# placeforyiming/DistanceTransform-DepthCompletion

Hardware: AMD Instinct MI355X
Metric: DT+NN-fill frames/sec at 352x1216; achieved HBM GB/s vs peak (higher is better)
Workload: dtype u32

## Files before the change

distancetransform-depthcompletion_amd/csrc/dtfill_fused.hpp:

```cpp
#pragma once

constexpr int F_NT = 256;
constexpr int F_P = 196;
constexpr int F_NWD = 6;
constexpr int F_HW = 3;
constexpr int F_RS = 7;
constexpr int F_RROWS = F_WHM + 4;
constexpr int F_RPLANE = F_RROWS * F_RS;
constexpr int F_RING = 1 + 4 * 2 * F_RPLANE;
constexpr int F_EB = 8;
constexpr int F_NONE = 2 * 63;
static_assert(F_WWM == 32 * F_NWD, "window width must be six words");
static_assert(F_RING * 4 >= F_WHM * F_P + 256 * 8, "s_par and the un-slicing table must fit in the ring's memory");
static_assert((F_WHM * F_P) % 8 == 0 && F_WHM * F_P >= 4 * (1 + 4 * F_RPLANE), "the table is 8-byte aligned and lies behind the planes of P1b");

template <int T, int ROW, int BACK>
__device__ __forceinline__ void tap_step(const u32 (&src)[5], u32 (&taken)[F_HW], u32 (&C)[6][F_HW]) {
    static_assert(T >= 0 && T < 8 && ROW == code_di(T) && BACK == code_weight(T), "tap T reads row r + di of level t - weight");
#pragma unroll
    for (int i = 0; i < F_HW; ++i) {
        const u32 cand = row_shift<code_dj(T)>(src + i);
        const u32 sel = cand & ~taken[i];
        taken[i] |= cand;
#pragma unroll
        for (int j = 0; j < 6; ++j)
            if (code_enc(T) & (1 << j)) C[j][i] |= sel;
    }
}

template <int T, int ROW>
__device__ __forceinline__ void bwd_tap(const u32 (&a0)[5], const u32 (&a1)[5], const u32 (&a2)[5], const u32 (&dv)[5],
                                        const u32 (&b0)[F_HW], const u32 (&b1)[F_HW], const u32 (&b2)[F_HW],
                                        u32 (&taken)[F_HW], u32 (&C)[6][F_HW]) {
    constexpr int CODE = T | 8, DJ = code_dj(CODE);
    static_assert(T >= 0 && T < 8 && ROW == code_di(CODE), "backward tap T reads row r - di");
#pragma unroll
    for (int i = 0; i < F_HW; ++i) {
        const u32 m = dist_match<code_weight(CODE)>(row_shift<DJ>(a0 + i), row_shift<DJ>(a1 + i), row_shift<DJ>(a2 + i), b0[i], b1[i], b2[i]) &
                      row_shift<DJ>(dv + i);
        const u32 sel = m & ~taken[i];
        taken[i] |= m;
#pragma unroll
        for (int j = 0; j < 6; ++j)
            if (code_enc(CODE) & (1 << j)) C[j][i] |= sel;
    }
}

__device__ __forceinline__ u32 mul_u24_opaque(u32 a, u32 b) {
    u32 r;
    asm("v_mul_u32_u24 %0, %1, %2" : "=v"(r) : "v"(a), "v"(b));
    return r;
}

#ifdef FUSED_PROF
constexpr int F_PROF_SLOTS = 8192;
__device__ unsigned long long g_fused_prof[F_PROF_SLOTS][16];
constexpr int F_TL_WAVES = 1 << 16, F_TL_EV = 32;
__device__ unsigned long long g_fused_tl[F_TL_WAVES][F_TL_EV];
__device__ __forceinline__ unsigned long long fprof_realtime() {
    unsigned long long t;
    __builtin_amdgcn_sched_barrier(0);
    asm volatile("s_memrealtime %0\n\ts_waitcnt lgkmcnt(0)" : "=s"(t) :: "memory");
    __builtin_amdgcn_sched_barrier(0);
    return t;
}
struct FusedProf {
    unsigned long long t[8] = {}, n[8] = {}, tprev = __builtin_readcyclecounter();
    int nev = 0;
    __device__ int wave() const { return (blockIdx.y * gridDim.x + blockIdx.x) * (blockDim.x >> 6) + (threadIdx.x >> 6); }
    __device__ void event(int k) {
        const unsigned long long rt = fprof_realtime();
        if ((threadIdx.x & 63) == 0 && wave() < F_TL_WAVES && nev < F_TL_EV) g_fused_tl[wave()][nev] = rt << 4 | (unsigned)k;
        ++nev;
    }
    __device__ FusedProf() { event(15); }
    __device__ void mark(int k) {
        const unsigned long long t_ = __builtin_readcyclecounter();
        t[k] += t_ - tprev;
        tprev = t_;
        event(k);
    }
    __device__ void flush() {
        const int slot = wave() % F_PROF_SLOTS;
        if ((threadIdx.x & 63) == 0)
            for (int k = 0; k < 8; ++k) {
                atomicAdd(&g_fused_prof[slot][k], t[k]);
                atomicAdd(&g_fused_prof[slot][8 + k], n[k]);
            }
    }
};
#define FPROF(...) __VA_ARGS__
#else
#define FPROF(...)
#endif

__device__ __forceinline__ void ring_load5(const u32 *__restrict__ ring, int slot, int plane, int row, int wb,
                                           u32 (&a)[5]) {
    const u32 *p = ring + 1 + (slot * 2 + plane) * F_RPLANE + row * F_RS + wb - 1;
#pragma unroll
    for (int i = 0; i < 5; ++i) a[i] = p[i];
}
__device__ __forceinline__ void ring_store3(u32 *__restrict__ ring, int slot, int plane, int row, int wb,
                                            const u32 (&w)[F_HW]) {
    u32 *p = ring + 1 + (slot * 2 + plane) * F_RPLANE + row * F_RS + wb;
#pragma unroll
    for (int i = 0; i < F_HW; ++i) p[i] = w[i];
}

template <int FR, int NT, bool EPI, bool STREAM>
__device__ __forceinline__ bool fused_walk_epilogue(
    const u8 *__restrict__ s_par, const short *__restrict__ s_tab, const uint2 *__restrict__ s_rw, int b, int H,
    int W, int th, int tw, int r0, int c0, int wr0, int wc0, int sh, const float *__restrict__ x,
    const float *__restrict__ vlist,
    int *__restrict__ finfo, int nval, int misaligned, int sky0, float *__restrict__ out_depth, float *__restrict__ out_dt,
    int32_t *__restrict__ out_index, int *__restrict__ frame_status, const DepthEpilogue ep, u32 *__restrict__ rowflag
    FPROF(, FusedProf &prof)) {
    const size_t fo = (size_t)b * H * W;
    const float *gbase = misaligned ? vlist + fo : x + fo;
    const u32 dcrop = EPI ? (u32)(ep.row0 * W) << 2 : 0u;
    const u32 tbytes = (u32)((r0 + th) * W) << 2;
    auto uni = [](int v) { return __builtin_amdgcn_readfirstlane(v); };
    const auto rs_d = __builtin_amdgcn_make_buffer_rsrc(out_depth ? out_depth + (size_t)b * (H - ep.row0) * W : nullptr, 0,
                                                        uni(out_depth && tbytes > dcrop ? (int)(tbytes - dcrop) : 0), 0x00020000);
    const auto rs_t = __builtin_amdgcn_make_buffer_rsrc(out_dt ? out_dt + fo : nullptr, 0, uni(out_dt ? (int)tbytes : 0), 0x00020000);
    const auto rs_i = __builtin_amdgcn_make_buffer_rsrc(out_index ? out_index + fo : nullptr, 0, uni(out_index ? (int)tbytes : 0), 0x00020000);
    constexpr u32 OFF_NONE = 0x80000000u;
    const char *tab = reinterpret_cast<const char *>(s_tab);
    auto step_of = [&](int c) { return (int)*reinterpret_cast<const short *>(tab + c); };
    const int src_base = wr0 * W + wc0;
    const int wrest = W - F_P;
    const u32 last_px = (u32)(H * W - 1);
    bool overflow = false;
    auto put = [](__amdgpu_buffer_rsrc_t rs, u32 off, u32 v) { __builtin_amdgcn_raw_buffer_store_b32(v, rs, (int)off, 0, STREAM ? 2 : 0); };
    const int nslots = ((th + F_EB - 1) / F_EB) * tw;
    const float inv_tw = 1.0f / (float)tw;
    const u32 w4 = (u32)W << 2;
    float p_val[F_EB];
#pragma unroll
    for (int e = 0; e < F_EB; ++e) p_val[e] = 0.0f;
    u32 p_o[F_EB];
#pragma unroll
    for (int e = 0; e < F_EB; ++e) p_o[e] = OFF_NONE;
    auto retire = [&]() {
#pragma unroll
        for (int e = 0; e < F_EB; ++e) put(rs_d, p_o[e] - dcrop, __float_as_uint(EPI ? depth_epilogue(p_val[e], ep) : p_val[e]));
    };
    for (int sb = 0; sb < nslots; sb += NT) {
        int pos[F_EB], step[F_EB], code[F_EB];
        u32 o[F_EB], home0;
        FPROF(prof.mark(5); ++prof.n[2]);
        {
            const int L = sb + (int)threadIdx.x, Lc = min(L, nslots - 1);
            const int g = (int)(((float)Lc + 0.5f) * inv_tw);
            const int tc = Lc - __mul24(g, tw), trb = g * F_EB;
            home0 = (u32)(FR + trb) << 16 | (u32)(FR + tc);
            u32 op = L < nslots ? (u32)(__mul24(r0 + trb, W) + c0 + tc) << 2 : OFF_NONE;
            const int pos0 = __mul24(FR + trb, F_P) + FR + tc;
            unsigned long long und = 0;
#pragma unroll
            for (int e = 0; e < F_EB; ++e) {
                pos[e] = pos0 + e * F_P;
                code[e] = s_par[pos[e]];
                und |= __ballot(code[e] == F_NONE);
                o[e] = code[e] != F_NONE ? op : OFF_NONE;
                asm volatile("" : "+v"(o[e]), "+v"(op));
                op += w4;
            }
            if (und) {
                const int nv = L < nslots ? th - trb : 0;
#pragma unroll
                for (int e = 0; e < F_EB; ++e) overflow |= e < nv && code[e] == F_NONE;
            }
        }
        for (int hop = 0; hop < FR + 2; hop += 2) {
#pragma unroll
            for (int e = 0; e < F_EB; ++e) step[e] = step_of(code[e]);
            int moving = 0;
#pragma unroll
            for (int e = 0; e < F_EB; ++e) moving |= step[e];
            if (!__any(moving != 0)) break;
            FPROF(++prof.n[5]);
#pragma unroll
            for (int e = 0; e < F_EB; ++e) pos[e] += step[e];
#pragma unroll
            for (int e = 0; e < F_EB; ++e) code[e] = s_par[pos[e]];
#pragma unroll
            for (int e = 0; e < F_EB; ++e) step[e] = step_of(code[e]);
#pragma unroll
            for (int e = 0; e < F_EB; ++e) pos[e] += step[e];
#pragma unroll
            for (int e = 0; e < F_EB; ++e) code[e] = s_par[pos[e]];
        }
        FPROF(prof.mark(4); for (int e = 0; e < F_EB; ++e) prof.n[3] += __popcll(__ballot(o[e] != OFF_NONE)));
        int pr[F_EB];
        u32 rc[F_EB], goff[F_EB];
        int lab[F_EB];
        constexpr int F_RG = 4;
#pragma unroll
        for (int h = 0; h < F_EB; h += F_RG) {
            int bp[F_RG], ri[F_RG];
            uint2 rw[F_RG];
            static_assert(F_P == 196 && F_WHM * F_P < (1 << 15), "the reciprocal below is F_P's");
#pragma unroll
            for (int k = 0; k < F_RG; ++k) {
                const int e = h + k;
                pr[e] = (int)(__umul24((u32)pos[e], 5350u) >> 20);
                rc[e] = __umul24((u32)pr[e], 65536u - F_P) + (u32)pos[e];
                bp[k] = (int)(rc[e] + (u32)sh);
                ri[k] = pr[e] * 8 + (int)__builtin_amdgcn_ubfe((u32)bp[k], 5u, 3u);
            }
#pragma unroll
            for (int k = 0; k < F_RG; ++k) rw[k] = s_rw[ri[k]];
#pragma unroll
            for (int k = 0; k < F_RG; ++k) lab[h + k] = (int)rw[k].y + __popc(__builtin_amdgcn_ubfe(rw[k].x, 0u, (u32)bp[k]));
        }
        if (!misaligned) {
#pragma unroll
            for (int e = 0; e < F_EB; ++e) {
                u32 t = (u32)(__mul24(pr[e], wrest) + pos[e]);
                asm("" : "+v"(t));
                goff[e] = min((t + (u32)src_base) << 2, last_px << 2);
            }
        } else {
            bool bad = false;
            const int nv = th + FR - (int)(home0 >> 16);
#pragma unroll
            for (int e = 0; e < F_EB; ++e) {
                const DepthIndex di = depth_index_pos(lab[e], nval);
                bad |= o[e] != OFF_NONE && e < nv && !di.ok;
                goff[e] = (di.ok ? min((u32)di.idx, last_px) : 0u) << 2;
            }
            if (bad && out_depth) atomicOr(frame_status + b, DTFILL_FRAME_INDEX_ERROR);
        }
        retire();
#pragma unroll
        for (int e = 0; e < F_EB; ++e) p_val[e] = *reinterpret_cast<const float *>(reinterpret_cast<const char *>(gbase) + goff[e]);
#pragma unroll
        for (int e = 0; e < F_EB; ++e) {
            p_o[e] = o[e];
            put(rs_i, o[e], (u32)lab[e]);
            put(rs_t, o[e], __float_as_uint((float)__builtin_amdgcn_sad_u16(rc[e], home0 + ((u32)e << 16), 0u)));
        }
    }
    FPROF(prof.mark(5));
    retire();
    const bool any = __any(overflow);
    if (any && !EPI) {
        for (int L = threadIdx.x; L < nslots; L += NT) {
            const int g = L / tw, tc = L - g * tw;
            for (int tr = g * F_EB; tr < min(g * F_EB + F_EB, th); ++tr)
                if (s_par[__mul24(FR + tr, F_P) + FR + tc] == F_NONE) {
                    rowflag[(size_t)b * H + r0 + tr] = 1u;
                    if (sky0 > 0 && (r0 + tr == sky0 || r0 + tr == sky0 + 1)) atomicOr(&finfo[b * FI_STRIDE + FI_SKY], SKY_OFF);
                }
        }
    }
    return any;
}

template <int FR, bool EPI, bool STREAM>
__device__ __forceinline__ void fused_body(int tile, bool premarked, int tbase, int nval, int misaligned, int sky0, const u32 *__restrict__ s_bs,
    const u32 *__restrict__ s_far,
    const float *__restrict__ x, const u64 *__restrict__ srcbits, const u16 *__restrict__ wpre_s,
    const u32 *__restrict__ rowbase_s, int *__restrict__ finfo, const float *__restrict__ vlist,
    int H, int W, int Wd, int nty, int TW, int tiles_x, float *__restrict__ out_depth,
    float *__restrict__ out_dt, int32_t *__restrict__ out_index,
    int *__restrict__ fflag, u32 *__restrict__ rowfar, int *__restrict__ frame_status, const DepthEpilogue ep, u32 *__restrict__ s_ring, uint2 *__restrict__ s_rw,
    short *__restrict__ s_tab, u32 (*__restrict__ s_any)[F_NT / 64]) {
    const int tid = threadIdx.x;
    const int b = blockIdx.x;
    const int ty = tile / tiles_x, tx = tile - ty * tiles_x;
    const int TH = tile_row_height(H, tbase, nty);
    int r0 = tbase + ty * TH;
    const int c0 = tx * TW;
    int th = min(TH, H - r0);
    const int tw = min(TW, W - c0);
    if (th <= 0) return;
    if (premarked) {
        const u32 *rowflag = rowfar + (size_t)b * H;
        auto mine = [&](int i) { return s_far ? ((s_far[i >> 5] >> (i & 31)) & 1u) == 0u : rowflag[i] == 0u; };
        if (tid == 0) {
            s_any[0][0] = 0xFFFFFFFFu;
            s_any[0][1] = 0u;
        }
        __syncthreads();
        if (tid < th && mine(r0 + tid)) {
            atomicMin(&s_any[0][0], (u32)tid);
            atomicMax(&s_any[0][1], (u32)tid + 1u);
        }
        __syncthreads();
        const u32 lo = s_any[0][0], hi = s_any[0][1];
        if (hi == 0u) return;
        r0 += (int)lo;
        th = (int)(hi - lo);
    }
    FPROF(FusedProf prof; prof.n[0] = 1);
    const int wr0 = r0 - FR, wc0 = c0 - FR;
    const int WH = th + 2 * FR, WW = tw + 2 * FR;
    const int ca = max(0, -wc0), cb = min(WW, W - wc0);
    const int w0 = wc0 >> 6;
    const int sh = wc0 - 64 * w0;

    const int r = tid & (F_WHM - 1);
    const int hf = tid >> 7;
    const int wb = F_HW * hf;
    u32 M[F_HW], D[F_HW], TM[F_HW];
    {
        const int gi = wr0 + r;
        const bool rowin = r < WH && gi >= 0 && gi < H;
        const int bit0 = sh + 96 * hf;
        const int kw = bit0 >> 6;
        u32 g[7];
#pragma unroll
        for (int k = 0; k < 3; ++k) {
            const int kk = kw + k;
            const int w = w0 + kk;
            u64 sb = 0;
            u32 rk = 0;
            if (rowin && kk < 4 && w >= 0 && w < Wd) {
                const size_t wi = ((size_t)b * H + gi) * Wd + w;
                sb = srcbits[wi];
                rk = (s_bs ? s_bs[gi] : rowbase_s[(size_t)b * H + gi]) + wpre_s[wi];
            }
            g[2 * k] = (u32)sb;
            g[2 * k + 1] = (u32)(sb >> 32);
            const bool mine = hf == 0 ? kk < 2 : (kk >= 2 && kk < 4);
            if (mine) {
                s_rw[r * 8 + 2 * kk] = make_uint2((u32)sb, rk + 1u);
                s_rw[r * 8 + 2 * kk + 1] = make_uint2((u32)(sb >> 32), rk + 1u + (u32)__popc((u32)sb));
            }
        }
        g[6] = 0;
        const int s6 = bit0 & 63;
        const bool hi = s6 & 32;
        const int s5 = s6 & 31;
#pragma unroll
        for (int i = 0; i < F_HW; ++i) {
            const u32 lo_w = hi ? g[i + 1] : g[i], hi_w = hi ? g[i + 2] : g[i + 1];
            const u32 word = s5 ? __builtin_amdgcn_alignbit(hi_w, lo_w, s5) : lo_w;
            const int lo = max(ca - 32 * (wb + i), 0), up = min(cb - 32 * (wb + i), 32);
            u32 m = 0;
            if (rowin && up > lo) m = (up >= 32 ? 0xFFFFFFFFu : ((1u << up) - 1u)) & ~((1u << lo) - 1u);
            M[i] = m;
            D[i] = word & m;
            const int tlo = max(FR - 32 * (wb + i), 0), tup = min(FR + tw - 32 * (wb + i), 32);
            u32 tm = 0;
            if (r >= FR && r < FR + th && tup > tlo) tm = (tup >= 32 ? 0xFFFFFFFFu : ((1u << tup) - 1u)) & ~((1u << tlo) - 1u);
            TM[i] = tm;
        }
    }
    if (s_bs) __syncthreads();
    for (int k = tid; k < F_RING; k += F_NT) s_ring[k] = 0;
    if (tid < 64) {
        const int hi = tid >> 3, lo = tid & 7;
        s_tab[tid] = (hi <= 4 && lo <= 4) ? (short)((hi - 2) * F_P + (lo - 2)) : (short)0;
    }
    __syncthreads();
    ring_store3(s_ring, 0, 0, r + 2, wb, D);
    ring_store3(s_ring, 0, 1, r + 2, wb, D);
    u32 C[6][F_HW];
#pragma unroll
    for (int j = 0; j < 6; ++j)
#pragma unroll
        for (int i = 0; i < F_HW; ++i) C[j][i] = ((18 >> j) & 1) ? D[i] : 0u;
    u32 Dup[F_HW], Ddn[F_HW];
    u32 Dl = 0, Dr = 0;
#pragma unroll
    for (int i = 0; i < F_HW; ++i) Dup[i] = Ddn[i] = 0;
    __syncthreads();
    FPROF(prof.mark(0));

    u32 P0[F_HW], P1[F_HW], P2[F_HW];
#pragma unroll
    for (int i = 0; i < F_HW; ++i) P0[i] = P1[i] = P2[i] = 0;
    for (int t = 1; t <= FR; ++t) {
        FPROF(++prof.n[1]);
        const int s1 = (t - 1) & 3, s2 = (t - 2) & 3, s3 = (t - 3) & 3, sw = t & 3;
        u32 nb[5], e1[5], l1[5], taken[F_HW], Et[F_HW], Lt[F_HW];
        ring_load5(s_ring, s1, 0, r + 2, wb, e1);
        Dl |= e1[0];
        Dr |= e1[4];
        ring_load5(s_ring, s1, 0, r + 1, wb, nb);
#pragma unroll
        for (int i = 0; i < F_HW; ++i) Dup[i] |= nb[i + 1];
        u32 e1d[5];
        ring_load5(s_ring, s1, 0, r + 3, wb, e1d);
        bool nonempty = false;
        {
            const u32 dd[5] = {Dl, D[0], D[1], D[2], Dr};
#pragma unroll
            for (int i = 0; i < F_HW; ++i) {
                Ddn[i] |= e1d[i + 1];
                const u32 dil = row_shift<1>(dd + i) | row_shift<-1>(dd + i) | Dup[i] | Ddn[i];
                Et[i] = dil & ~D[i] & M[i];
                taken[i] = ~Et[i];
                nonempty |= Et[i] != 0;
            }
        }
        ring_load5(s_ring, s3, 1, r + 0, wb, nb);
        tap_step<0, -2, 3>(nb, taken, C);
        tap_step<1, -2, 3>(nb, taken, C);
        {
            u32 l3[5], l2[5];
            ring_load5(s_ring, s3, 1, r + 1, wb, l3);
            ring_load5(s_ring, s2, 1, r + 1, wb, l2);
            ring_load5(s_ring, s1, 1, r + 1, wb, nb);
            tap_step<2, -1, 3>(l3, taken, C);
            tap_step<3, -1, 2>(l2, taken, C);
            tap_step<4, -1, 1>(nb, taken, C);
            tap_step<5, -1, 2>(l2, taken, C);
            tap_step<6, -1, 3>(l3, taken, C);
        }
        ring_load5(s_ring, s1, 1, r + 2, wb, l1);
        tap_step<7, 0, 1>(l1, taken, C);
        {
            const u32 m0 = (t & 1) ? 0xFFFFFFFFu : 0u, m1 = (t & 2) ? 0xFFFFFFFFu : 0u, m2 = (t & 4) ? 0xFFFFFFFFu : 0u;
#pragma unroll
            for (int i = 0; i < F_HW; ++i) {
                Lt[i] = taken[i] & Et[i];
                P0[i] |= Et[i] & m0;
                P1[i] |= Et[i] & m1;
                P2[i] |= Et[i] & m2;
            }
        }
#pragma unroll
        for (int i = 0; i < F_HW; ++i) D[i] |= Et[i];
        ring_store3(s_ring, sw, 0, r + 2, wb, Et);
        ring_store3(s_ring, sw, 1, r + 2, wb, Lt);
        {
            bool open = false;
#pragma unroll
            for (int i = 0; i < F_HW; ++i) open |= (TM[i] & ~D[i]) != 0;
            const u32 flags = (__any(nonempty) ? 1u : 0u) | (__any(open) ? 2u : 0u);
            if ((tid & 63) == 0) s_any[t & 1][tid >> 6] = flags;
            __syncthreads();
            u32 any = 0;
#pragma unroll
            for (int w = 0; w < F_NT / 64; ++w) any |= s_any[t & 1][w];
            if (any != 3u) break;
        }
    }
    FPROF(prof.mark(1));
    __syncthreads();
    uint2 *s_lut = reinterpret_cast<uint2 *>(reinterpret_cast<u8 *>(s_ring) + F_WHM * F_P);
    s_lut[tid] = make_uint2((((u32)tid & 15u) * 0x00204081u) & 0x01010101u, (((u32)tid >> 4) * 0x00204081u) & 0x01010101u);
    ring_store3(s_ring, 0, 0, r + 2, wb, P0);
    ring_store3(s_ring, 0, 1, r + 2, wb, P1);
    ring_store3(s_ring, 1, 0, r + 2, wb, P2);
    ring_store3(s_ring, 1, 1, r + 2, wb, D);
    __syncthreads();
    {
        u32 taken[F_HW], a0[5], a1[5], a2[5], dv[5];
#pragma unroll
        for (int i = 0; i < F_HW; ++i) {
            const u32 live = C[0][i] | C[1][i] | C[2][i] | C[3][i] | C[4][i] | C[5][i];
            taken[i] = ~(D[i] & ~live);
        }
        auto row4 = [&](int row) {
            ring_load5(s_ring, 0, 0, row, wb, a0);
            ring_load5(s_ring, 0, 1, row, wb, a1);
            ring_load5(s_ring, 1, 0, row, wb, a2);
            ring_load5(s_ring, 1, 1, row, wb, dv);
        };
        row4(r + 4);
        bwd_tap<0, 2>(a0, a1, a2, dv, P0, P1, P2, taken, C);
        bwd_tap<1, 2>(a0, a1, a2, dv, P0, P1, P2, taken, C);
        row4(r + 3);
        bwd_tap<2, 1>(a0, a1, a2, dv, P0, P1, P2, taken, C);
        bwd_tap<3, 1>(a0, a1, a2, dv, P0, P1, P2, taken, C);
        bwd_tap<4, 1>(a0, a1, a2, dv, P0, P1, P2, taken, C);
        bwd_tap<5, 1>(a0, a1, a2, dv, P0, P1, P2, taken, C);
        bwd_tap<6, 1>(a0, a1, a2, dv, P0, P1, P2, taken, C);
        row4(r + 2);
        bwd_tap<7, 0>(a0, a1, a2, dv, P0, P1, P2, taken, C);
    }

    FPROF(prof.mark(2));
    u8 *s_par = reinterpret_cast<u8 *>(s_ring);
    __syncthreads();
    {
        u32 *prow = reinterpret_cast<u32 *>(s_par + r * F_P) + wb * 8;
#pragma unroll
        for (int i = 0; i < F_HW; ++i) {
            u32 cj[6];
#pragma unroll
            for (int j = 0; j < 6; ++j) cj[j] = C[j][i] | ~D[i];
#pragma unroll
            for (int q = 0; q < 4; ++q) {
                u32 lo = 0, hi = 0;
#pragma unroll
                for (int j = 0; j < 6; ++j) {
                    const uint2 sp = s_lut[(cj[j] >> (8 * q)) & 0xFFu];
                    lo |= sp.x << (j + 1);
                    hi |= sp.y << (j + 1);
                }
                prow[i * 8 + 2 * q] = lo;
                prow[i * 8 + 2 * q + 1] = hi;
            }
        }
    }
    __syncthreads();
    FPROF(prof.mark(3));

    const bool overflow = fused_walk_epilogue<FR, F_NT, EPI, STREAM>(s_par, s_tab, s_rw, b, H, W, th, tw, r0, c0, wr0, wc0, sh, x, vlist,
                                                        finfo, nval, misaligned, sky0, out_depth, out_dt, out_index, frame_status, ep, rowfar FPROF(, prof));
    if (overflow && (threadIdx.x & 63) == 0) {
        fflag[b] = EPI ? 2 : 1;
        atomicOr(frame_status + b, DTFILL_FRAME_GENERAL_PATH);
    }
    FPROF(prof.mark(6); prof.flush());
}

constexpr size_t F_OFF_RW = (sizeof(u32) * F_RING + 15) & ~(size_t)15, F_OFF_TAB = F_OFF_RW + sizeof(uint2) * F_WHM * 8, F_OFF_ANY = F_OFF_TAB + sizeof(short) * 64,
                 F_LDS_OWN = F_OFF_ANY + sizeof(u32) * 2 * (F_NT / 64);
constexpr size_t F_LDS = F_LDS_OWN;
constexpr int F_RIDE_HMAX = (int)((sizeof(u32) * F_RING - sizeof(FrameScratch)) / (2 * sizeof(u32)));
static_assert(sizeof(FrameScratch) % 4 == 0 && F_NT == 256, "frame_facts runs on the window kernel's 256 threads");

template <bool STREAM, bool EPI>
__global__ __launch_bounds__(F_NT, 4) void k_fused(
    const float *__restrict__ x, const u64 *__restrict__ srcbits, const u16 *__restrict__ wpre_s,
    const u32 *__restrict__ rowbase_s, int *__restrict__ finfo, float *vlist ,
    int H, int W, int Wd, FusedTiles t16, FusedTiles t32, float *__restrict__ out_depth,
    float *__restrict__ out_dt, int32_t *__restrict__ out_index,
    int *__restrict__ route, int *__restrict__ fflag, u32 *__restrict__ rowfar, int *__restrict__ frame_status, const DepthEpilogue ep,
    const FrameArgs fa) {
    __shared__ __attribute__((aligned(16))) unsigned char s_raw[F_LDS];
    u32 *s_ring = reinterpret_cast<u32 *>(s_raw);
    uint2 *s_rw = reinterpret_cast<uint2 *>(s_raw + F_OFF_RW);
    short *s_tab = reinterpret_cast<short *>(s_raw + F_OFF_TAB);
    u32(*s_any)[F_NT / 64] = reinterpret_cast<u32(*)[F_NT / 64]>(s_raw + F_OFF_ANY);
    const int b = blockIdx.x, tile = blockIdx.y;
    int rt, tbase, nval, misaligned, sky0;
    const u32 *s_bs = nullptr, *s_far = nullptr;
    if (fa.ride) {
        if (tile >= fa.ntmin) {
            if (threadIdx.x == 0) s_any[0][0] = (u32)__hip_atomic_load(&route[b], __ATOMIC_RELAXED, __HIP_MEMORY_SCOPE_AGENT);
            __syncthreads();
            const int seen = (int)s_any[0][0];
            const int rs = seen > 0 ? (seen & 0xFF) : 0;
            if (seen != ROUTE_UNKNOWN && !((rs == 16 && tile < t16.ntiles) || (rs == 32 && tile < t32.ntiles))) return;
        }
        FrameScratch &sc = *reinterpret_cast<FrameScratch *>(s_raw);
        u32 *bs = reinterpret_cast<u32 *>(s_raw + sizeof(FrameScratch)), *bv = bs + H;
        u32 *gs = fa.rowbase_s + (size_t)b * H, *gv = fa.rowbase_v + (size_t)b * H;
        const bool pub = tile == 0;
        const FrameFacts ff = frame_facts(fa.rowcnt_s + (size_t)b * H, fa.rowcnt_v + (size_t)b * H, H, W, fa.mode, fa.nty16, fa.nty32, sc, pub,
                                          [&](int i, u32 base_s, u32 base_v) {
                                              bs[i] = base_s;
                                              bv[i] = base_v;
                                              if (pub) {
                                                  gs[i] = base_s;
                                                  gv[i] = base_v;
                                              }
                                          });
        if (pub)
            frame_publish(ff, sc, b, fa.x, fa.valbits, fa.wpre_v, fa.srcbits, fa.wpre_s, fa.ptslist, H, W, Wd, gs, gv, finfo, vlist,
                          fflag, route, frame_status, fa.mode, fa.negflag, rowfar, true);
        else if (ff.misaligned && out_depth && ((ff.r == 16 && tile < t16.ntiles) || (ff.r == 32 && tile < t32.ntiles)))
            value_list(b, fa.x, fa.valbits, fa.wpre_v, H, W, Wd, vlist, [&](int i) { return bv[i]; });
        auto uni = [](int v) { return __builtin_amdgcn_readfirstlane(v); };
        rt = uni(ff.route);
        tbase = uni(ff.tr0);
        nval = uni(ff.nval);
        misaligned = uni(ff.misaligned);
        sky0 = uni(ff.sky);
        s_bs = bs;
        s_far = sc.far[ff.plane];
    } else {
        rt = route[b];
        tbase = finfo[b * FI_STRIDE + FI_TR0];
        nval = finfo[b * FI_STRIDE + FI_NVAL];
        misaligned = finfo[b * FI_STRIDE + FI_MISALIGNED];
        sky0 = finfo[b * FI_STRIDE + FI_SKY] & ~SKY_OFF;
    }
    if (rt == ROUTE_POINTS) return;
    const int r = rt > 0 ? (rt & 0xFF) : 0;
    const bool pre = rt > 0 && (rt & ROUTE_PREMARK);
#define FUSED_CALL(FR_, T_)                                                                                        \
    fused_body<FR_, EPI, STREAM>(tile, pre, tbase, nval, misaligned, sky0, s_bs, s_far, x, srcbits, wpre_s, rowbase_s, finfo, vlist, H, W, Wd, T_.nty, T_.TW, T_.tiles_x, out_depth, out_dt, \
                          out_index, fflag, rowfar, frame_status, ep, s_ring, s_rw, s_tab, s_any)
    if (r == 16 && tile < t16.ntiles)
        FUSED_CALL(16, t16);
    else if (r == 32 && tile < t32.ntiles)
        FUSED_CALL(32, t32);
#undef FUSED_CALL
}
```

distancetransform-depthcompletion_amd/csrc/dtfill_taps.hpp:

```cpp
#pragma once

constexpr int TAP_OFFSET[8][2] = {{-2, -1}, {-2, 1}, {-1, -2}, {-1, -1}, {-1, 0}, {-1, 1}, {-1, 2}, {0, -1}};
constexpr int tap_di(int t) { return TAP_OFFSET[t][0]; }
constexpr int tap_dj(int t) { return TAP_OFFSET[t][1]; }

constexpr bool code_fwd(int code) { return !(code & 8); }
constexpr int code_di(int code) { return code_fwd(code) ? tap_di(code & 7) : -tap_di(code & 7); }
constexpr int code_dj(int code) { return code_fwd(code) ? tap_dj(code & 7) : -tap_dj(code & 7); }
constexpr int code_weight(int code) { return (code_di(code) < 0 ? -code_di(code) : code_di(code)) + (code_dj(code) < 0 ? -code_dj(code) : code_dj(code)); }
constexpr int code_enc(int code) { return (code_di(code) + 2) << 3 | (code_dj(code) + 2); }

constexpr unsigned tap_nibbles(int axis, int t = 0) { return t == 8 ? 0u : (unsigned)(TAP_OFFSET[t][axis] + 2) << (4 * t) | tap_nibbles(axis, t + 1); }
constexpr unsigned TAP_DI_NIB = tap_nibbles(0), TAP_DJ_NIB = tap_nibbles(1);

constexpr void tap_decode(int code, int &di, int &dj) {
    const int sh = (code & 7) * 4;
    di = (int)((TAP_DI_NIB >> sh) & 15u) - 2;
    dj = (int)((TAP_DJ_NIB >> sh) & 15u) - 2;
    if (code & 8) {
        di = -di;
        dj = -dj;
    }
}
```

Before: 419,800.

## Shrink parent-code planes from six bits to four and drop redundant backward taps

Parent pointers are now stored as 4-bit tap codes (16 values) instead of 6-bit (di,dj) encodings. Codes 13 and 14 are reserved for source and undecided, which frees two bit-planes per word in registers and in the un-slicing epilogue. A separate live mask replaces the OR over all planes. Backward taps 5 and 6 are removed because their candidates are shown to be dominated by code 12. The goal is lower register pressure and fewer ALU and LDS lookups, at the cost of a decode table for codes and a correctness argument that rests on the static asserts.

```diff
diff --git a/distancetransform-depthcompletion_amd/csrc/dtfill_fused.hpp b/distancetransform-depthcompletion_amd/csrc/dtfill_fused.hpp
--- a/distancetransform-depthcompletion_amd/csrc/dtfill_fused.hpp
+++ b/distancetransform-depthcompletion_amd/csrc/dtfill_fused.hpp
@@ -8,32 +8,36 @@
 constexpr int F_RROWS = F_WHM + 4;
 constexpr int F_RPLANE = F_RROWS * F_RS;
 constexpr int F_RING = 1 + 4 * 2 * F_RPLANE;
+constexpr int F_NPLANES = 4;
 constexpr int F_EB = 8;
-constexpr int F_NONE = 2 * 63;
+constexpr int F_NONE = 2 * CODE_NONE;
+static_assert(CODE_SOURCE < (1 << F_NPLANES) && CODE_NONE < (1 << F_NPLANES) && !code_wins(CODE_SOURCE) && !code_wins(CODE_NONE), "the reserved codes fit the planes and never win");
 static_assert(F_WWM == 32 * F_NWD, "window width must be six words");
 static_assert(F_RING * 4 >= F_WHM * F_P + 256 * 8, "s_par and the un-slicing table must fit in the ring's memory");
 static_assert((F_WHM * F_P) % 8 == 0 && F_WHM * F_P >= 4 * (1 + 4 * F_RPLANE), "the table is 8-byte aligned and lies behind the planes of P1b");
 
 template <int T, int ROW, int BACK>
-__device__ __forceinline__ void tap_step(const u32 (&src)[5], u32 (&taken)[F_HW], u32 (&C)[6][F_HW]) {
+__device__ __forceinline__ void tap_step(const u32 (&src)[5], u32 (&taken)[F_HW], u32 (&C)[F_NPLANES][F_HW]) {
     static_assert(T >= 0 && T < 8 && ROW == code_di(T) && BACK == code_weight(T), "tap T reads row r + di of level t - weight");
+    static_assert(code_wins(T), "a reserved code is no tap");
 #pragma unroll
     for (int i = 0; i < F_HW; ++i) {
         const u32 cand = row_shift<code_dj(T)>(src + i);
         const u32 sel = cand & ~taken[i];
         taken[i] |= cand;
 #pragma unroll
-        for (int j = 0; j < 6; ++j)
-            if (code_enc(T) & (1 << j)) C[j][i] |= sel;
+        for (int j = 0; j < F_NPLANES; ++j)
+            if (plane_code(T) & (1 << j)) C[j][i] |= sel;
     }
 }
 
 template <int T, int ROW>
 __device__ __forceinline__ void bwd_tap(const u32 (&a0)[5], const u32 (&a1)[5], const u32 (&a2)[5], const u32 (&dv)[5],
                                         const u32 (&b0)[F_HW], const u32 (&b1)[F_HW], const u32 (&b2)[F_HW],
-                                        u32 (&taken)[F_HW], u32 (&C)[6][F_HW]) {
+                                        u32 (&taken)[F_HW], u32 (&C)[F_NPLANES][F_HW]) {
     constexpr int CODE = T | 8, DJ = code_dj(CODE);
     static_assert(T >= 0 && T < 8 && ROW == code_di(CODE), "backward tap T reads row r - di");
+    static_assert(code_wins(CODE), "codes 13 and 14 never select (dtfill_taps.hpp): they mean source and undecided here");
 #pragma unroll
     for (int i = 0; i < F_HW; ++i) {
         const u32 m = dist_match<code_weight(CODE)>(row_shift<DJ>(a0 + i), row_shift<DJ>(a1 + i), row_shift<DJ>(a2 + i), b0[i], b1[i], b2[i]) &
@@ -41,8 +45,8 @@
         const u32 sel = m & ~taken[i];
         taken[i] |= m;
 #pragma unroll
-        for (int j = 0; j < 6; ++j)
-            if (code_enc(CODE) & (1 << j)) C[j][i] |= sel;
+        for (int j = 0; j < F_NPLANES; ++j)
+            if (plane_code(CODE) & (1 << j)) C[j][i] |= sel;
     }
 }
 
@@ -351,18 +355,22 @@
     }
     if (s_bs) __syncthreads();
     for (int k = tid; k < F_RING; k += F_NT) s_ring[k] = 0;
-    if (tid < 64) {
-        const int hi = tid >> 3, lo = tid & 7;
-        s_tab[tid] = (hi <= 4 && lo <= 4) ? (short)((hi - 2) * F_P + (lo - 2)) : (short)0;
+    if (tid < (1 << F_NPLANES)) {
+        int di, dj;
+        code_step(tid, di, dj);
+        s_tab[tid] = (short)(di * F_P + dj);
     }
     __syncthreads();
     ring_store3(s_ring, 0, 0, r + 2, wb, D);
     ring_store3(s_ring, 0, 1, r + 2, wb, D);
-    u32 C[6][F_HW];
-#pragma unroll
-    for (int j = 0; j < 6; ++j)
-#pragma unroll
-        for (int i = 0; i < F_HW; ++i) C[j][i] = ((18 >> j) & 1) ? D[i] : 0u;
+    u32 C[F_NPLANES][F_HW];
+    u32 Lv[F_HW];
+#pragma unroll
+    for (int i = 0; i < F_HW; ++i) {
+        Lv[i] = D[i];
+#pragma unroll
+        for (int j = 0; j < F_NPLANES; ++j) C[j][i] = ((CODE_SOURCE >> j) & 1) ? D[i] : 0u;
+    }
     u32 Dup[F_HW], Ddn[F_HW];
     u32 Dl = 0, Dr = 0;
 #pragma unroll
@@ -373,7 +381,7 @@
     u32 P0[F_HW], P1[F_HW], P2[F_HW];
 #pragma unroll
     for (int i = 0; i < F_HW; ++i) P0[i] = P1[i] = P2[i] = 0;
-    for (int t = 1; t <= FR; ++t) {
+    auto level = [&](const int t) __attribute__((always_inline)) -> bool {
         FPROF(++prof.n[1]);
         const int s1 = (t - 1) & 3, s2 = (t - 2) & 3, s3 = (t - 3) & 3, sw = t & 3;
         u32 nb[5], e1[5], l1[5], taken[F_HW], Et[F_HW], Lt[F_HW];
@@ -418,6 +426,7 @@
 #pragma unroll
             for (int i = 0; i < F_HW; ++i) {
                 Lt[i] = taken[i] & Et[i];
+                Lv[i] |= Lt[i];
                 P0[i] |= Et[i] & m0;
                 P1[i] |= Et[i] & m1;
                 P2[i] |= Et[i] & m2;
@@ -437,9 +446,10 @@
             u32 any = 0;
 #pragma unroll
             for (int w = 0; w < F_NT / 64; ++w) any |= s_any[t & 1][w];
-            if (any != 3u) break;
-        }
-    }
+            return any == 3u;
+        }
+    };
+    for (int t = 1; t <= FR && level(t); ++t) {}
     FPROF(prof.mark(1));
     __syncthreads();
     uint2 *s_lut = reinterpret_cast<uint2 *>(reinterpret_cast<u8 *>(s_ring) + F_WHM * F_P);
@@ -452,10 +462,7 @@
     {
         u32 taken[F_HW], a0[5], a1[5], a2[5], dv[5];
 #pragma unroll
-        for (int i = 0; i < F_HW; ++i) {
-            const u32 live = C[0][i] | C[1][i] | C[2][i] | C[3][i] | C[4][i] | C[5][i];
-            taken[i] = ~(D[i] & ~live);
-        }
+        for (int i = 0; i < F_HW; ++i) taken[i] = ~(D[i] & ~Lv[i]);
         auto row4 = [&](int row) {
             ring_load5(s_ring, 0, 0, row, wb, a0);
             ring_load5(s_ring, 0, 1, row, wb, a1);
@@ -469,8 +476,6 @@
         bwd_tap<2, 1>(a0, a1, a2, dv, P0, P1, P2, taken, C);
         bwd_tap<3, 1>(a0, a1, a2, dv, P0, P1, P2, taken, C);
         bwd_tap<4, 1>(a0, a1, a2, dv, P0, P1, P2, taken, C);
-        bwd_tap<5, 1>(a0, a1, a2, dv, P0, P1, P2, taken, C);
-        bwd_tap<6, 1>(a0, a1, a2, dv, P0, P1, P2, taken, C);
         row4(r + 2);
         bwd_tap<7, 0>(a0, a1, a2, dv, P0, P1, P2, taken, C);
     }
@@ -482,14 +487,14 @@
         u32 *prow = reinterpret_cast<u32 *>(s_par + r * F_P) + wb * 8;
 #pragma unroll
         for (int i = 0; i < F_HW; ++i) {
-            u32 cj[6];
-#pragma unroll
-            for (int j = 0; j < 6; ++j) cj[j] = C[j][i] | ~D[i];
+            u32 cj[F_NPLANES];
+#pragma unroll
+            for (int j = 0; j < F_NPLANES; ++j) cj[j] = ((CODE_NONE >> j) & 1) ? C[j][i] | ~D[i] : C[j][i];
 #pragma unroll
             for (int q = 0; q < 4; ++q) {
                 u32 lo = 0, hi = 0;
 #pragma unroll
-                for (int j = 0; j < 6; ++j) {
+                for (int j = 0; j < F_NPLANES; ++j) {
                     const uint2 sp = s_lut[(cj[j] >> (8 * q)) & 0xFFu];
                     lo |= sp.x << (j + 1);
                     hi |= sp.y << (j + 1);
@@ -511,7 +516,7 @@
     FPROF(prof.mark(6); prof.flush());
 }
 
-constexpr size_t F_OFF_RW = (sizeof(u32) * F_RING + 15) & ~(size_t)15, F_OFF_TAB = F_OFF_RW + sizeof(uint2) * F_WHM * 8, F_OFF_ANY = F_OFF_TAB + sizeof(short) * 64,
+constexpr size_t F_OFF_RW = (sizeof(u32) * F_RING + 15) & ~(size_t)15, F_OFF_TAB = F_OFF_RW + sizeof(uint2) * F_WHM * 8, F_OFF_ANY = F_OFF_TAB + sizeof(short) * (1 << F_NPLANES),
                  F_LDS_OWN = F_OFF_ANY + sizeof(u32) * 2 * (F_NT / 64);
 constexpr size_t F_LDS = F_LDS_OWN;
 constexpr int F_RIDE_HMAX = (int)((sizeof(u32) * F_RING - sizeof(FrameScratch)) / (2 * sizeof(u32)));
diff --git a/distancetransform-depthcompletion_amd/csrc/dtfill_taps.hpp b/distancetransform-depthcompletion_amd/csrc/dtfill_taps.hpp
--- a/distancetransform-depthcompletion_amd/csrc/dtfill_taps.hpp
+++ b/distancetransform-depthcompletion_amd/csrc/dtfill_taps.hpp
@@ -22,3 +22,34 @@
         dj = -dj;
     }
 }
+
+static_assert(code_di(12) == 1 && code_dj(12) == 0 && code_weight(12) == 1, "code 12 steps one row down");
+static_assert(code_di(13) == 1 && code_di(14) == 1, "codes 13 and 14 read the row that code 12 reads");
+static_assert((code_dj(13) < 0 ? -code_dj(13) : code_dj(13)) == code_weight(13) - 1 &&
+              (code_dj(14) < 0 ? -code_dj(14) : code_dj(14)) == code_weight(14) - 1, "their candidates lie weight - 1 beside code 12's");
+constexpr int plane_code(int code) { return code; }
+constexpr int CODE_SOURCE = 13;
+constexpr int CODE_NONE = 14;
+constexpr bool code_wins(int code) { return code != CODE_SOURCE && code != CODE_NONE; }
+
+struct CodeStepTable {
+    int v[16][2];
+    constexpr CodeStepTable() : v{} {
+        for (int c = 0; c < 16; ++c) {
+            v[c][0] = code_wins(c) ? code_di(c) : 0;
+            v[c][1] = code_wins(c) ? code_dj(c) : 0;
+        }
+    }
+};
+constexpr CodeStepTable CODE_STEP{};
+constexpr void code_step(int code, int &di, int &dj) {
+    tap_decode(code, di, dj);
+    if (!code_wins(code)) di = dj = 0;
+}
+constexpr bool code_step_agrees(int c = 0) {
+    int di = 9, dj = 9;
+    if (c == 16) return true;
+    code_step(c, di, dj);
+    return di == CODE_STEP.v[c][0] && dj == CODE_STEP.v[c][1] && code_step_agrees(c + 1);
+}
+static_assert(code_step_agrees(), "code_step and CODE_STEP are one table");
```

Result: faster. 427,400, median of 6 (+1.8%).
